# NIH-NEI/oct-image-segmentation-models

Measured on AMD Instinct MI355X. Metric: B-scans/sec (train step), 256x512 3-class U-Net, higher is better.
Workload: dtype f32; 1 GPU; configs[1]: train step (fwd+Dice-macro+bwd+allreduce+Adam), per-GPU batch 32, 256x512x1, 3-class, pool_layers=4, start_neurons=8, random-init weights; global_batch=32, parallelism=dp1, allreduce=none

## Files before the change

oct-image-segmentation-models_amd/csrc/common.hpp:

```cpp
#pragma once
#include <hip/hip_runtime.h>
#include <stdint.h>

namespace oct {

constexpr int kTileX = 32;
constexpr int kTileY = 8;
constexpr int kBlock = 256;

enum { BN_A = 0, BN_B = 1, BN_MEAN = 2, BN_RSTD = 3, BN_C1 = 4, BN_C2 = 5, BN_GA = 6, BN_GB = 7, BN_GD = 8, BN_ARRAYS = 9 };

enum { F_U8 = 1, F_AFF = 2, F_TWO = 4, F_UP = 8, F_DROP = 16 };

static __constant__ float c_u8_lut[256];

__host__ __device__ inline uint32_t drop_hash(uint64_t seed, uint64_t step, uint32_t idx) {
    uint64_t x = seed ^ (step * 0x9E3779B97F4A7C15ull) ^ ((uint64_t)idx * 0xD1B54A32D192ED03ull);
    x ^= x >> 33; x *= 0xff51afd7ed558ccdull;
    x ^= x >> 33; x *= 0xc4ceb9fe1a85ec53ull;
    x ^= x >> 33;
    return (uint32_t)(x >> 32);
}

struct DropCfg {
// ... 101 lines not shown
template <> struct Raw4<float> { using type = float4; };
template <> struct Raw4<bf16_t> { using type = uint2; };
template <typename AT> __device__ inline typename Raw4<AT>::type ldraw4(const AT* p);
template <> __device__ inline float4 ldraw4<float>(const float* p) { return *reinterpret_cast<const float4*>(p); }
template <> __device__ inline uint2 ldraw4<bf16_t>(const bf16_t* p) { return *reinterpret_cast<const uint2*>(p); }
template <typename AT> __device__ inline typename Raw4<AT>::type raw_zero4();
template <> __device__ inline float4 raw_zero4<float>() { return make_float4(0.f, 0.f, 0.f, 0.f); }
template <> __device__ inline uint2 raw_zero4<bf16_t>() { return make_uint2(0u, 0u); }
__device__ inline float4 widen4(const float4& r) { return r; }
__device__ inline float4 widen4(const uint2& u) {
    return make_float4(__uint_as_float(u.x << 16), __uint_as_float(u.x & 0xFFFF0000u),
                       __uint_as_float(u.y << 16), __uint_as_float(u.y & 0xFFFF0000u));
}
template <typename AT> __device__ inline void sta4(AT* p, const float4& v);
template <> __device__ inline void sta4<float>(float* p, const float4& v) { *reinterpret_cast<float4*>(p) = v; }
typedef __bf16 bf16x2_hw __attribute__((ext_vector_type(2)));
typedef float f32x2_hw __attribute__((ext_vector_type(2)));
template <> __device__ inline void sta4<bf16_t>(bf16_t* p, const float4& v) {
    uint2 u;
    u.x = __builtin_bit_cast(uint32_t, __builtin_convertvector(f32x2_hw{v.x, v.y}, bf16x2_hw));
    u.y = __builtin_bit_cast(uint32_t, __builtin_convertvector(f32x2_hw{v.z, v.w}, bf16x2_hw));
    *reinterpret_cast<uint2*>(p) = u;
}
template <typename AT> __device__ inline float lda1(const AT* p);
template <> __device__ inline float lda1<float>(const float* p) { return *p; }
template <> __device__ inline float lda1<bf16_t>(const bf16_t* p) { return bf2f(*p); }

}
```

oct-image-segmentation-models_amd/csrc/host.hpp:

```cpp
#pragma once
#include <hip/hip_runtime.h>

#include <string>
#include <vector>

#include "common.hpp"
#include "kernels_bwd.hpp"
#include "kernels_igemm.hpp"

namespace octh {

struct Options {
    int thin_min_tiles = 2048;
    int dw32_blocks = 512, dw16_blocks = 768;
    int igemm_p_blocks = 1280;
    int igemm_min_blocks = 512;
    int dwpair8 = 1;
    int pair_geo = 221;
    int pair_min_tiles = 2048;
    int dw_side_stream = 1;
    int bx_two_blocks = 1;
    int bx_waves = 8;
    int fuse_first_apply = 1;
    int fuse_bn_apply = 1;
    int fuse_bn_apply16 = 1;
    int fuse_dw_thin = 1;
    int timing_skip = 0;
    int fuse_bn_finalize = 0;
    int bt_m2 = 1;
    int dwbt_f32_all = 0;
    int bt_blocks_per_cu = 0;
    int dwbx_enable = 1;
    int dwbx_blocks = 256;
    int bx_min_blocks = 256;
    int mfma_mode = 1;
    int focal_clip_mod = 0;
    int fork_on_launch = 1;
    int dw_fork_group = 1;
    int event_sysfence = 0;
    int persist_min_tiles = 2048;
};
extern Options g_opt;

int fail(int code, const std::string& msg);

#define HIP_OK(expr)                                                                                      \
    do {                                                                                                  \
        hipError_t e__ = (expr);                                                                          \
        if (e__ != hipSuccess) return ::octh::fail(-5, std::string(#expr) + ": " + hipGetErrorString(e__)); \
    } while (0)

// ... 44 lines not shown
```

oct-image-segmentation-models_amd/csrc/kernels_bwd.hpp:

```cpp
#pragma once
#include "common.hpp"
#include "kernels_fwd.hpp"

namespace oct {

struct PoolBwdArgs {
    const void* gp;
    const void* z;
    const float* bn;
    void* g;
    float* part;
    int H, W, C, tiles_x, tiles, act_bf16;
    FinDesc fin;
};

template <int C_T, typename AT>
__global__ __launch_bounds__(kBlock) void pool_bwd_k(const PoolBwdArgs A) {
    __shared__ float red[256];
    const int Ho = A.H >> 1, Wo = A.W >> 1;
    const int tx = threadIdx.x & (kTileX - 1), ty = threadIdx.x / kTileX;
    const int tile = blockIdx.x;
    const int xo = (tile % A.tiles_x) * kTileX + tx, yo = (tile / A.tiles_x) * kTileY + ty;
    const int b = blockIdx.z, c0 = blockIdx.y * C_T;
    const bool valid = xo < Wo && yo < Ho;
// ... 27 lines not shown
                yv[q] = fmaxf(fmaf(a, zv[q][i], bb), 0.f);
                if (yv[q] > best) { best = yv[q]; am = q; }
            }
#pragma unroll
            for (int q = 0; q < 4; ++q) {
                const float gt = yv[q] > 0.f ? gd[q][i] + (q == am ? gpv[i] : 0.f) : 0.f;
                s1[i] += gt; s2[i] += gt * ((zv[q][i] - mean) * rstd);
                gd[q][i] = gt;
            }
        }
#pragma unroll
        for (int q = 0; q < 4; ++q)
#pragma unroll
            for (int i = 0; i < C_T; i += 4) sta4<AT>(Ag + off[q] + i, make_float4(gd[q][i], gd[q][i + 1], gd[q][i + 2], gd[q][i + 3]));
    }
    float* out = A.part + ((size_t)b * A.tiles + tile) * (2 * A.C);
    block_reduce_store<C_T>(s1, red, out + c0, C_T);
    block_reduce_store<C_T>(s2, red, out + A.C + c0, C_T);
}

template <typename AT, int V = 4>
__global__ __launch_bounds__(kBlock) void pool_bwd_flat_k(const PoolBwdArgs A, int B) {
    static_assert(V == 4 || V == 8, "channels per thread");
    __shared__ float sh[4 * 64 * 8];
    const int CV = A.C / V, Ho = A.H >> 1, Wo = A.W >> 1;
    const size_t n = (size_t)B * Ho * Wo * CV;
    const int tid = threadIdx.x, lane = tid & 63, wave = tid >> 6, c = V * (tid % CV);
    float a[V], bb[V], mean[V], rstd[V], s1[V], s2[V];
#pragma unroll
    for (int k = 0; k < V; ++k) {
        a[k] = A.bn[BN_A * A.C + c + k]; bb[k] = A.bn[BN_B * A.C + c + k];
        mean[k] = A.bn[BN_MEAN * A.C + c + k]; rstd[k] = A.bn[BN_RSTD * A.C + c + k];
        s1[k] = 0.f; s2[k] = 0.f;
    }
    const AT* Az = reinterpret_cast<const AT*>(A.z); AT* Ag = reinterpret_cast<AT*>(A.g);
    const AT* Agp = reinterpret_cast<const AT*>(A.gp);
    for (size_t i = (size_t)blockIdx.x * kBlock + tid; i < n; i += (size_t)gridDim.x * kBlock) {
        size_t r = i / CV;
        const int xo = (int)(r % Wo); r /= Wo;
        const int yo = (int)(r % Ho); const int b = (int)(r / Ho);
        float gpv[V];
        size_t off[4]; float zv[4][V], gd[4][V];
        const size_t goff = (((size_t)b * Ho + yo) * Wo + xo) * A.C + c;
#pragma unroll
        for (int j = 0; j < V; j += 4) {
            const float4 gq = lda4<AT>(Agp + goff + j);
            gpv[j] = gq.x; gpv[j + 1] = gq.y; gpv[j + 2] = gq.z; gpv[j + 3] = gq.w;
// ... 280 lines not shown
#pragma unroll
                for (int kx = 0; kx < KW; ++kx)
                    acc[ky * KW + kx] = fmaf(Xs[((py + ky) * XW + pxx + kx) * CI_T + ci], d, acc[ky * KW + kx]);
        }
    }
#pragma unroll
    for (int k = 0; k < TAPS; ++k) Rs[t * (TAPS + 1) + k] = acc[k];
    Rs[t * (TAPS + 1) + TAPS] = accb;
    __syncthreads();
    if (t < NT) {
        const size_t wsize = (size_t)TAPS * A.Cin * A.Cout;
        float* out = A.part + (size_t)blockIdx.x * (wsize + A.Cout);
        const bool ok = (ci0 + ci < A.Cin) && (co0 + co < A.Cout);
        for (int k = 0; k <= TAPS; ++k) {
            float s = 0.f;
            for (int q = 0; q < PS; ++q) s += Rs[(q * NT + t) * (TAPS + 1) + k];
            if (!ok) continue;
            if (k < TAPS) out[((size_t)k * A.Cin + ci0 + ci) * A.Cout + co0 + co] = s;
            else if (ci0 + ci == 0) out[wsize + co0 + co] = s;
        }
    }
}

template <typename AT, bool FUSE>
__global__ __launch_bounds__(kBlock) void conv_dw_first_k(const ConvBwdWArgs A, int tiles_x, int tiles, int total_tiles) {
    constexpr int TH = 8, TW = 128, XH = TH + 2, XW = TW + 2;
    __shared__ float Xs[XH * XW];
    __shared__ float red[256];
    __shared__ float lut_s[256];
    const int t = threadIdx.x, xl = t & 31, row = t >> 5;
    lut_s[t] = c_u8_lut[t];
    float acc0[64], acc1[16];
#pragma unroll
    for (int k = 0; k < 64; ++k) acc0[k] = 0.f;
#pragma unroll
    for (int k = 0; k < 16; ++k) acc1[k] = 0.f;
    const bool u8 = (A.flags & F_U8) != 0;
    for (int tl = blockIdx.x; tl < total_tiles; tl += gridDim.x) {
        const int b = tl / tiles, tile = tl % tiles;
        const int x0 = (tile % tiles_x) * TW, y0 = (tile / tiles_x) * TH;
        __syncthreads();
        {
            constexpr int NS = (XH * XW + kBlock - 1) / kBlock;
            unsigned int rb[NS]; float rf[NS]; bool in[NS];
#pragma unroll
            for (int k = 0; k < NS; ++k) {
                const int i = t + k * kBlock, cy = i / XW, cx = i % XW, iy = y0 + cy - 1, ix = x0 + cx - 1;
                in[k] = i < XH * XW && iy >= 0 && iy < A.H && ix >= 0 && ix < A.W;
                const size_t pix = in[k] ? ((size_t)b * A.H + iy) * A.W + ix : 0;
                rb[k] = 0; rf[k] = 0.f;
                if (in[k]) { if (u8) rb[k] = reinterpret_cast<const unsigned char*>(A.x0)[pix]; else rf[k] = reinterpret_cast<const float*>(A.x0)[pix]; }
            }
#pragma unroll
            for (int k = 0; k < NS; ++k) {
                const int i = t + k * kBlock;
                if (i < XH * XW) Xs[i] = in[k] ? (u8 ? lut_s[rb[k]] : rf[k]) : 0.f;
            }
        }
        __syncthreads();
        const int y = y0 + row;
#pragma unroll
        for (int k = 0; k < TW / 32; ++k) {
            const int xx = xl + 32 * k, x = x0 + xx;
            if (y < A.H && x < A.W) {
                const size_t e8 = (((size_t)b * A.H + y) * A.W + x) * 8;
                const AT* dp = reinterpret_cast<const AT*>(A.dz) + e8;
                const float4 d0 = lda4<AT>(dp), d1 = lda4<AT>(dp + 4);
                float d[8] = {d0.x, d0.y, d0.z, d0.w, d1.x, d1.y, d1.z, d1.w};
                if constexpr (FUSE) {
                    const AT* zp = reinterpret_cast<const AT*>(A.zf) + e8;
                    const float4 z0 = lda4<AT>(zp), z1 = lda4<AT>(zp + 4);
                    const float zv[8] = {z0.x, z0.y, z0.z, z0.w, z1.x, z1.y, z1.z, z1.w};
#pragma unroll
                    for (int co = 0; co < 8; ++co) {
                        const float o = bn_bwd_apply1(A.bnf[BN_GA * 8 + co], A.bnf[BN_GB * 8 + co], A.bnf[BN_GD * 8 + co], d[co], zv[co]);
                        d[co] = dz_as_stored<AT>(o);
                        asm volatile("" : "+v"(d[co]));
                    }
                }
#pragma unroll
                for (int tap = 0; tap < 9; ++tap) {
                    const float xv = Xs[(row + tap / 3) * XW + xx + tap % 3];
#pragma unroll
                    for (int co = 0; co < 8; ++co) {
                        if (tap < 8) acc0[tap * 8 + co] = fmaf(xv, d[co], acc0[tap * 8 + co]);
                        else acc1[co] = fmaf(xv, d[co], acc1[co]);
                    }
                }
#pragma unroll
                for (int co = 0; co < 8; ++co) acc1[8 + co] += d[co];
            }
        }
    }
    float* out = A.part + (size_t)blockIdx.x * 80;
    block_reduce_store<64>(acc0, red, out, 64);
    block_reduce_store<16>(acc1, red, out + 64, 16);
}

// ... 75 lines not shown
```

oct-image-segmentation-models_amd/csrc/kernels_fin.hpp:

```cpp
#pragma once
#include "common.hpp"

namespace oct {

struct FinDesc {
    unsigned* counter;
    int bwd;
    double count;
    float* bn;
    const float* gamma; const float* beta;
    float* mm; float* mv; float eps, momentum; int unbiased;
    float* dgamma; float* dbeta;
};

__device__ __forceinline__ void bn_fwd_finalize_write(double s, double q, double count, int C, int c, float* __restrict__ bn,
                                                      const float* __restrict__ gamma, const float* __restrict__ beta,
                                                      float* __restrict__ mm, float* __restrict__ mv, float eps, float momentum,
                                                      int unbiased) {
    const double mean = s / count;
    double var = q / count - mean * mean;
    if (var < 0) var = 0;
    const double rstd = 1.0 / sqrt(var + (double)eps);
    const double a = (double)gamma[c] * rstd;
    bn[BN_A * C + c] = (float)a;
    bn[BN_B * C + c] = (float)((double)beta[c] - mean * a);
    bn[BN_MEAN * C + c] = (float)mean;
    bn[BN_RSTD * C + c] = (float)rstd;
    const double m = momentum;
    const double uv = (unbiased && count > 1) ? var * (count / (count - 1.0)) : var;
    mm[c] = (float)((double)mm[c] * m + mean * (1.0 - m));
    mv[c] = (float)((double)mv[c] * m + uv * (1.0 - m));
}

__device__ __forceinline__ void bn_bwd_finalize_write(double s, double q, double count, int C, int c, float* __restrict__ bn,
                                                      const float* __restrict__ gamma, float* __restrict__ dgamma,
                                                      float* __restrict__ dbeta) {
    dbeta[c] = (float)s;
    dgamma[c] = (float)q;
    const double c1 = s / count, c2 = q / count;
    const double rstd = (double)bn[BN_RSTD * C + c], mean = (double)bn[BN_MEAN * C + c];
    const double ga = (double)gamma[c] * rstd, gb = -ga * rstd * c2, gd = -ga * c1 - gb * mean;
    bn[BN_C1 * C + c] = (float)c1; bn[BN_C2 * C + c] = (float)c2;
    bn[BN_GA * C + c] = (float)ga; bn[BN_GB * C + c] = (float)gb; bn[BN_GD * C + c] = (float)gd;
}

__device__ __forceinline__ void part_store(float* p, float v) { __hip_atomic_store(p, v, __ATOMIC_RELAXED, __HIP_MEMORY_SCOPE_AGENT); }

__device__ inline void finalize_in_launch(const FinDesc& F, const float* __restrict__ part, int rows, int C, unsigned nblocks, char* lds) {
    asm volatile("s_waitcnt vmcnt(0)" ::: "memory");
    __syncthreads();
    int* const flag = reinterpret_cast<int*>(lds);
    if (threadIdx.x == 0) {
        const unsigned prev = __hip_atomic_fetch_add(F.counter, 1u, __ATOMIC_RELAXED, __HIP_MEMORY_SCOPE_AGENT);
        *flag = prev == nblocks - 1 ? 1 : 0;
    }
    __syncthreads();
    if (*flag) {
        double* const sh = reinterpret_cast<double*>(lds + 16);
        double* const tot = sh + 2 * (size_t)blockDim.x;
        const int Wp = C, G = (int)blockDim.x / Wp, t = threadIdx.x;
        if (t < G * Wp) {
            const int q = t % Wp, g = t / Wp;
            const unsigned long long* col = reinterpret_cast<const unsigned long long*>(part) + q;
            double s0 = 0, s1 = 0;
            int r = g;
            for (; r + 31 * G < rows; r += 32 * G) {
                unsigned long long v[32];
#pragma unroll
                for (int k = 0; k < 32; ++k) v[k] = __hip_atomic_load(col + (size_t)(r + k * G) * Wp, __ATOMIC_RELAXED, __HIP_MEMORY_SCOPE_AGENT);
#pragma unroll
                for (int k = 0; k < 32; ++k) { s0 += (double)__uint_as_float((unsigned)v[k]); s1 += (double)__uint_as_float((unsigned)(v[k] >> 32)); }
            }
            for (; r + 7 * G < rows; r += 8 * G) {
                unsigned long long v[8];
#pragma unroll
                for (int k = 0; k < 8; ++k) v[k] = __hip_atomic_load(col + (size_t)(r + k * G) * Wp, __ATOMIC_RELAXED, __HIP_MEMORY_SCOPE_AGENT);
// ... 2 lines not shown
            }
            for (; r < rows; r += G) {
                const unsigned long long v = __hip_atomic_load(col + (size_t)r * Wp, __ATOMIC_RELAXED, __HIP_MEMORY_SCOPE_AGENT);
                s0 += (double)__uint_as_float((unsigned)v); s1 += (double)__uint_as_float((unsigned)(v >> 32));
            }
            sh[2 * t] = s0; sh[2 * t + 1] = s1;
        }
        __syncthreads();
        if (t < 2 * C) {
            double a = 0;
            for (int g = 0; g < G; ++g) a += sh[2 * (g * Wp + (t >> 1)) + (t & 1)];
            tot[t] = a;
        }
        __syncthreads();
        if (t < C) {
            if (F.bwd) bn_bwd_finalize_write(tot[t], tot[C + t], F.count, C, t, F.bn, F.gamma, F.dgamma, F.dbeta);
            else bn_fwd_finalize_write(tot[t], tot[C + t], F.count, C, t, F.bn, F.gamma, F.beta, F.mm, F.mv, F.eps, F.momentum, F.unbiased);
        }
        if (t == 0) __hip_atomic_store(F.counter, 0u, __ATOMIC_RELAXED, __HIP_MEMORY_SCOPE_AGENT);
    }
    __syncthreads();
}

}
```

oct-image-segmentation-models_amd/csrc/kernels_fwd.hpp:

```cpp
#pragma once
#include "common.hpp"
#include "kernels_fin.hpp"

namespace oct {

struct ConvFwdArgs {
    const void* x0;
    const float* ab0;
    int C0;
    const float* x1;
    const float* ab1;
    int C1;
    const float* w;
    const float* bias;
    void* z;
    float* part;
    int H, W, Cin, Cout, tiles_x, tiles;
    DropCfg drop;
    int act_bf16;
    FinDesc fin;
};

template <int CO_T, int FLAGS>
__device__ inline void accum_src(const void* __restrict__ src, const float* __restrict__ ab, int C, size_t pix,
// ... 66 lines not shown
            const int sy = UP ? iy >> 1 : iy, sx = UP ? ix >> 1 : ix;
            const size_t pix = inb ? ((size_t)b * Hs + sy) * Ws + sx : 0;
            const float* wk = A.w + (size_t)((ky * KW + kx) * A.Cin) * A.Cout + co0;
            accum_src<CO_T, FLAGS>(A.x0, A.ab0, A.C0, pix, inb, wk, A.Cout, A.drop, acc);
            if constexpr (TWO)
                accum_src<CO_T, FLAGS>(A.x1, A.ab1, A.C1, pix, inb, wk + (size_t)A.C0 * A.Cout, A.Cout, A.drop, acc);
        }
    }
    if (valid) {
        AT* zp = reinterpret_cast<AT*>(A.z) + (((size_t)b * A.H + y) * A.W + x) * A.Cout + co0;
#pragma unroll
        for (int j = 0; j < CO_T; j += 4) sta4<AT>(zp + j, make_float4(acc[j], acc[j + 1], acc[j + 2], acc[j + 3]));
    }
    if (A.part) {
        float s[CO_T], q[CO_T];
#pragma unroll
        for (int j = 0; j < CO_T; ++j) { s[j] = valid ? acc[j] : 0.f; q[j] = s[j] * s[j]; }
        float* out = A.part + ((size_t)b * A.tiles + tile) * (2 * A.Cout);
        block_reduce_store<CO_T>(s, red, out + co0, CO_T);
        block_reduce_store<CO_T>(q, red, out + A.Cout + co0, CO_T);
    }
}

template <typename AT>
__global__ __launch_bounds__(kBlock) void conv_first_fwd_k(const ConvFwdArgs A, int x_is_u8, int tiles_x, int tiles, int total_tiles,
                                                          const float* __restrict__ wgt, const float* __restrict__ bias) {
    constexpr int TH = 8, TW = 128, XH = TH + 2, XW = TW + 2;
    __shared__ float Xs[XH * XW];
    __shared__ float red[256];
    __shared__ float lut_s[256];
    const int t = threadIdx.x, xl = t & 31, row = t >> 5;
    lut_s[t] = c_u8_lut[t];
    float s1[8], s2[8];
#pragma unroll
    for (int j = 0; j < 8; ++j) { s1[j] = 0.f; s2[j] = 0.f; }
    for (int tl = blockIdx.x; tl < total_tiles; tl += gridDim.x) {
        const int b = tl / tiles, tile = tl % tiles;
        const int x0 = (tile % tiles_x) * TW, y0 = (tile / tiles_x) * TH;
        __syncthreads();
        {
            constexpr int NS = (XH * XW + kBlock - 1) / kBlock;
            unsigned int rb[NS]; float rf[NS]; bool in[NS];
#pragma unroll
            for (int k = 0; k < NS; ++k) {
                const int i = t + k * kBlock, cy = i / XW, cx = i % XW, iy = y0 + cy - 1, ix = x0 + cx - 1;
                in[k] = i < XH * XW && iy >= 0 && iy < A.H && ix >= 0 && ix < A.W;
                const size_t pix = in[k] ? ((size_t)b * A.H + iy) * A.W + ix : 0;
                rb[k] = 0; rf[k] = 0.f;
                if (in[k]) { if (x_is_u8) rb[k] = reinterpret_cast<const unsigned char*>(A.x0)[pix]; else rf[k] = reinterpret_cast<const float*>(A.x0)[pix]; }
            }
#pragma unroll
            for (int k = 0; k < NS; ++k) {
                const int i = t + k * kBlock;
                if (i < XH * XW) Xs[i] = in[k] ? (x_is_u8 ? lut_s[rb[k]] : rf[k]) : 0.f;
            }
        }
        __syncthreads();
        const int y = y0 + row;
#pragma unroll
        for (int k = 0; k < TW / 32; ++k) {
            const int xx = xl + 32 * k, x = x0 + xx;
            float acc[8];
#pragma unroll
            for (int j = 0; j < 8; ++j) acc[j] = bias[j];
#pragma unroll
            for (int tap = 0; tap < 9; ++tap) {
                const float xv = Xs[(row + tap / 3) * XW + xx + tap % 3];
#pragma unroll
                for (int j = 0; j < 8; ++j) acc[j] = fmaf(xv, wgt[tap * 8 + j], acc[j]);
            }
            if (y < A.H && x < A.W) {
                AT* zp = reinterpret_cast<AT*>(A.z) + (((size_t)b * A.H + y) * A.W + x) * 8;
                sta4<AT>(zp, make_float4(acc[0], acc[1], acc[2], acc[3]));
                sta4<AT>(zp + 4, make_float4(acc[4], acc[5], acc[6], acc[7]));
#pragma unroll
                for (int j = 0; j < 8; ++j) { s1[j] += acc[j]; s2[j] = fmaf(acc[j], acc[j], s2[j]); }
            }
        }
    }
    if (A.part) {
        float* out = A.part + (size_t)blockIdx.x * 16;
        block_reduce_store<8, true>(s1, red, out, 8);
        block_reduce_store<8, true>(s2, red, out + 8, 8);
        if (A.fin.counter) finalize_in_launch(A.fin, A.part, gridDim.x, 8, gridDim.x, reinterpret_cast<char*>(Xs));
    }
}

struct BnFinArgs {
    const float* part;
    int nblk, C;
    double count;
    const float* gamma; const float* beta;
    float* bn;
// ... 84 lines not shown
}

template <int C, int CIN>
__device__ inline void head_logits(const float* __restrict__ ab, const float* __restrict__ w, const float* __restrict__ bias,
                                   float (&y)[CIN], const float (&zr)[CIN], float (&p)[C]) {
#pragma unroll
    for (int i = 0; i < CIN; ++i) y[i] = fmaxf(fmaf(ab[i], zr[i], ab[CIN + i]), 0.f);
    float mx = -3.4e38f;
#pragma unroll
    for (int c = 0; c < C; ++c) {
        float l = bias[c];
#pragma unroll
        for (int i = 0; i < CIN; ++i) l = fmaf(y[i], w[i * C + c], l);
        p[c] = l; mx = fmaxf(mx, l);
    }
    float sum = 0.f;
#pragma unroll
    for (int c = 0; c < C; ++c) { p[c] = expf(p[c] - mx); sum += p[c]; }
    const float inv = 1.f / sum;
#pragma unroll
    for (int c = 0; c < C; ++c) p[c] *= inv;
}

template <int C, int CIN, typename AT>
__global__ __launch_bounds__(kBlock) void head_fwd_k(const HeadFwdArgs A) {
    constexpr int N = DiceN<C>::value;
    __shared__ float red[256];
    const int b = blockIdx.y;
    float v[N];
#pragma unroll
    for (int i = 0; i < N; ++i) v[i] = 0.f;
    for (int chunk = blockIdx.x; chunk * kBlock < A.HW; chunk += gridDim.x) {
        const int px = chunk * kBlock + threadIdx.x;
        const bool valid = px < A.HW;
        const size_t pix = (size_t)b * A.HW + (valid ? px : 0);
        float y[CIN], zr[CIN], p[C];
        head_load<CIN, AT>(reinterpret_cast<const AT*>(A.z) + pix * CIN, zr);
        head_logits<C, CIN>(A.ab, A.w, A.bias, y, zr, p);
        if (valid) {
            if (A.probs) {
#pragma unroll
                for (int c = 0; c < C; ++c) A.probs[pix * C + c] = p[c];
            }
            if (A.argmax) {
                int am = 0; float best = p[0];
#pragma unroll
                for (int c = 1; c < C; ++c) if (p[c] > best) { best = p[c]; am = c; }
                A.argmax[pix] = (unsigned char)am;
            }
            if (A.labels) {
                const int lab = A.labels[pix];
#pragma unroll
                for (int c = 0; c < C; ++c) {
                    const float yv = lab == c ? 1.f : 0.f, ph = p[c] > 0.5f ? 1.f : 0.f;
                    v[c * kDiceVals + 0] += yv * p[c]; v[c * kDiceVals + 1] += yv; v[c * kDiceVals + 2] += p[c];
                    v[c * kDiceVals + 3] += yv * ph;   v[c * kDiceVals + 4] += ph;
                }
                if (A.focal_on) {
                    float py = p[0];
#pragma unroll
                    for (int c = 1; c < C; ++c) py = lab == c ? p[c] : py;
// ... 113 lines not shown
```

oct-image-segmentation-models_amd/csrc/oct_unet.hip:

```cpp
#include <hip/hip_runtime.h>
#include <hip/hip_ext.h>

#include <cmath>
#include <cstdio>
#include <cstring>
#include <string>
#include <vector>

#include "../../include/oct_unet.h"
#include "host.hpp"
#include "kernels_bwd.hpp"
#include "kernels_fwd.hpp"
#include "kernels_igemm.hpp"
#include "kernels_bx.hpp"

using namespace oct;
using namespace octh;

#ifndef OCT_SRC_HASH
#define OCT_SRC_HASH "unstamped"
#endif

namespace octh {
Options g_opt;
// ... 247 lines not shown
    return off;
}

DropCfg make_drop(const oct_unet* h) {
    DropCfg d;
    d.seed = h->cfg.seed; d.step = h->drop_step;
    const double r = h->cfg.dropout_rate;
    d.thresh = (unsigned)std::min(4294967295.0, std::floor(r * 4294967296.0));
    d.scale = (float)(1.0 / (1.0 - r));
    return d;
}

inline bool fin_ok(const oct_unet* h, const Layer& l) { return h->opt.fuse_bn_finalize && l.has_bn && l.cout <= 32 && l.cout % 2 == 0; }
FinDesc fin_desc(const oct_unet* h, int li, int bwd, int B) {
    const Layer& l = h->plan.L[li];
    FinDesc f{};
    f.counter = h->fin_counters + 2 * li + (bwd ? 1 : 0); f.bwd = bwd; f.count = (double)B * l.H * l.W;
    f.bn = l.bn; f.gamma = h->params + l.gamma_off; f.beta = h->params + l.beta_off;
    f.mm = h->state + l.mm_off; f.mv = h->state + l.mv_off;
    f.eps = h->cfg.bn_eps; f.momentum = h->cfg.bn_momentum; f.unbiased = h->cfg.bn_unbiased_moving_var;
    if (bwd) { f.dgamma = h->grads + l.gamma_off; f.dbeta = h->grads + l.beta_off; }
    return f;
}

template <int KH, int FLAGS>
int launch_conv_fwd_co(const ConvFwdArgs& a, int B, hipStream_t s, const char* layer, double flops, double bytes) {
    const int co_t = chunk_of(a.Cout);
    dim3 grid(a.tiles, a.Cout / co_t, B), block(kBlock);
    char nm[64]; snprintf(nm, sizeof nm, "conv_fwd_k<%d,%d,%d,%s>", KH, co_t, FLAGS, AT_NAME(a.act_bf16));
    ProfScope ps(s, nm, layer, flops, bytes);
    switch (co_t) {
        case 16: AT_DISPATCH(a.act_bf16, conv_fwd_k<KH, 16, FLAGS, AT><<<grid, block, 0, s>>>(a)); break;
        case 8: AT_DISPATCH(a.act_bf16, conv_fwd_k<KH, 8, FLAGS, AT><<<grid, block, 0, s>>>(a)); break;
        default: AT_DISPATCH(a.act_bf16, conv_fwd_k<KH, 4, FLAGS, AT><<<grid, block, 0, s>>>(a)); break;
    }
    HIP_OK(hipGetLastError());
    return 0;
}

struct SrcDesc { const void* x0; const float* ab0; int C0; const void* x1; const float* ab1; int C1; int flags; };

SrcDesc src_of(const oct_unet* h, int li, const void* x_in, int x_is_u8) {
    const Layer& l = h->plan.L[li];
    SrcDesc d{}; d.x1 = nullptr; d.ab1 = nullptr; d.C1 = 0;
    switch (l.src) {
        case SRC_INPUT: d.x0 = x_in; d.ab0 = nullptr; d.C0 = l.cin; d.flags = x_is_u8 ? F_U8 : 0; break;
// ... 210 lines not shown
    e.jw = e.stride < 16384 ? 16 : 64;
    e.blk_start = R.n ? R.L[R.n - 1].blk_start + cdiv((int)R.L[R.n - 1].stride, R.L[R.n - 1].jw) : 0;
    ++R.n;
}

int flush_reduce(oct_unet* h, hipStream_t s) {
    ReduceAllArgs& R = h->red;
    if (!R.n) return 0;
    const ReduceAllArgs::Entry& last = R.L[R.n - 1];
    const unsigned blocks = last.blk_start + cdiv((int)last.stride, last.jw);
    double bytes = 0;
    for (int i = 0; i < R.n; ++i) bytes += (double)R.L[i].npb * R.L[i].stride * 4;
    ProfScope ps(s, "reduce_all_k", "all", 0, bytes);
    reduce_all_k<<<blocks, kBlock, 0, s>>>(R);
    HIP_OK(hipGetLastError());
    R.n = 0;
    return 0;
}

inline bool first_dw_streams(const Layer& l) {
    return l.src == SRC_INPUT && l.cin == 1 && l.cout == 8 && l.kh == 3 && l.has_bn && !l.drop_in;
}

int conv_backward_w(oct_unet* h, int li, const void* x_in, int x_is_u8, const void* dz, int B, hipStream_t s, bool fused_apply) {
    const Layer& l = h->plan.L[li];
    const Options& o = h->opt;
    const SrcDesc sd = src_of(h, li, x_in, x_is_u8);
    DwPlan p = dw_plan(l, B, o.mfma_mode, h->cfg.dtype, o);
    p.npb = std::min(p.npb, l.dw_rows);
    ConvBwdWArgs a{};
    a.x0 = sd.x0; a.ab0 = sd.ab0; a.C0 = sd.C0; a.x1 = sd.x1; a.ab1 = sd.ab1; a.C1 = sd.C1;
    a.flags = sd.flags | (l.drop_in ? F_DROP : 0);
    a.dz = dz; a.part = l.dwp;
    a.B = B; a.H = l.H; a.W = l.W; a.Cin = l.cin; a.Cout = l.cout;
    a.tiles_x = cdiv(l.W, kTileX); a.tiles = p.tiles; a.total_tiles = B * a.tiles; a.npb = p.npb;
    a.drop = make_drop(h); a.act_bf16 = h->cfg.dtype;
    if (fused_apply) { a.zf = l.z; a.bnf = l.bn; }
    const double px = (double)B * l.H * l.W, fl = 2.0 * l.kh * l.kw * l.cin * l.cout * px;
    const int es = h->cfg.dtype ? 2 : 4;
    const double by = in_bytes(l, B, x_is_u8, es) + px * l.cout * es * (fused_apply ? 2 : 1);
    const bool up = l.src == SRC_UP;
    const LaunchCtx lc{&o, B, s, l.name, fl, by};
    int rc = 0;
    if (p.kind == 0 && l.cin == 1 && l.cout == 8 && l.kh == 3 && !(a.flags & (F_AFF | F_DROP | F_TWO | F_UP))) {
        const int tx = cdiv(l.W, 128), tiles = tx * cdiv(l.H, 8), total = B * tiles;
        const int grid = std::min(total, a.npb);
        a.npb = grid;
        const int bf = a.act_bf16;
        ProfScope ps(s, bf ? "conv_dw_first_k<unsigned short>" : "conv_dw_first_k<float>", l.name, fl, by);
        if (fused_apply) AT_DISPATCH(bf, (conv_dw_first_k<AT, true><<<grid, kBlock, 0, s>>>(a, tx, tiles, total)));
        else AT_DISPATCH(bf, (conv_dw_first_k<AT, false><<<grid, kBlock, 0, s>>>(a, tx, tiles, total)));
        HIP_OK(hipGetLastError());
    } else if (p.kind == 0) {
        if (fused_apply) return fail(-3, "conv_backward_w: the generic first-layer kernel does not apply the BN-backward transform");
        rc = launch_dw<3>(a, p.cic, p.coc, s, l.name, fl, by);
    } else if (p.kind == 33 || p.kind == 34) {
        rc = launch_dw_bf16pipe(a, p, l.kh, up, lc);
    } else {
        rc = launch_dw_f32pipe(a, p, l.kh, up, lc);
    }
    if (rc) return rc;
    queue_reduce(h, l, a.npb);
    return 0;
}

int bn_backward(oct_unet* h, int li, int nblk, int B, hipStream_t s, bool finalize_only, bool finalized_in_launch,
                hipEvent_t done = nullptr, bool* bound = nullptr) {
    const Layer& l = h->plan.L[li];
    if (bound) *bound = false;
    if (!finalized_in_launch && !(h->opt.timing_skip & 2 && h->drop_step > 2)) {
        BnBwdFinArgs f{};
        f.part = h->stat_part; f.nblk = nblk; f.C = l.cout; f.count = (double)B * l.H * l.W;
        f.bn = l.bn; f.gamma = h->params + l.gamma_off; f.dgamma = h->grads + l.gamma_off; f.dbeta = h->grads + l.beta_off;
        ProfScope ps(s, "bn_bwd_finalize_k", l.name, 0, (double)nblk * 2 * l.cout * 4);
        if (done && finalize_only) {
            hipExtLaunchKernelGGL(bn_bwd_finalize_k, dim3(l.cout), dim3(kBlock), 0, s, nullptr, done, 0, f);
// ... 95 lines not shown
            fuse = o.fuse_first_apply && li == 0 && first_dw_streams(l) && dwkind == 0 &&
                   !(src_of(h, li, x_in, x_is_u8).flags & (F_AFF | F_DROP | F_TWO | F_UP));
        } else {
            const int cg = bx_bwd_cg(l);
            const bool up = l.src == SRC_UP;
            const ConvRoute r0 = conv_route(dx_args(nullptr, cg, 0, nullptr, up), up ? A_DOWN2 : A_NORMAL, o);
            fuse = o.fuse_bn_apply && dwkind != 0 && r0 != ROUTE_F32 && !(up && r0 == ROUTE_BX && l.cout > kBxGbDown2MaxC) &&
                   !(r0 == ROUTE_BT && l.cout == 32) && !(r0 == ROUTE_BT && l.cout == 16 && cg == 16 && !o.fuse_bn_apply16) &&
                   (l.src != SRC_CONCAT || conv_route(dx_args(nullptr, cg, cg, nullptr, false), A_NORMAL, o) != ROUTE_F32);
        }
        l.g_masked = fuse;
        bool fdw = false;
        if (fuse && o.fuse_dw_thin && l.kh == 3 && l.cout == 8 && !l.drop_in && (l.src == SRC_PREV || l.src == SRC_CONCAT) &&
            bx_bwd_cg(l) == 8 && l.dw_rows >= std::min(B * cdiv(l.W, 32) * cdiv(l.H, 8), 512) &&
            conv_route(dx_args(nullptr, 8, 0, nullptr, false), A_NORMAL, o) == ROUTE_BT &&
            (l.src != SRC_CONCAT || conv_route(dx_args(nullptr, 8, 8, nullptr, false), A_NORMAL, o) == ROUTE_BT))
            fdw = true;
        const bool fork = side_ok && !fdw && l.src != SRC_INPUT;
        const bool tail_here = li == first_mid_layer(pl);
        if (fork) pend.push_back({li, fuse});
        const bool flush = !pend.empty() && (!fork || (int)pend.size() >= o.dw_fork_group || tail_here);
        hipEvent_t fe = flush ? h->fork_ev[1 + n_forks++ % (h->fork_ev.size() - 1)] : nullptr;
        bool fe_bound = false;
        rc = bn_backward(h, li, pending_nblk, B, s, fuse, pending_fin, (flush && o.fork_on_launch) ? fe : nullptr, &fe_bound);
        if (rc) return rc;
        pending_fin = false;
        if (flush) {
            if (!fe_bound) HIP_OK(hipEventRecord(fe, s));
            HIP_OK(hipStreamWaitEvent(h->side, fe, 0));
            for (const PendingDw& p : pend) {
                rc = conv_backward_w(h, p.li, x_in, x_is_u8, pl.L[p.li].g, B, h->side, p.fuse);
                if (rc) return rc;
            }
            pend.clear();
            forked = true;
        }
        if (!fdw && !fork) {
            rc = conv_backward_w(h, li, x_in, x_is_u8, l.g, B, s, fuse);
            if (rc) return rc;
        }
        if (tail_here && (forked || h->tail_event)) {
            hipStream_t rs = forked ? h->side : s;
            rc = flush_reduce(h, rs);
            if (rc) return rc;
            if (h->tail_event) HIP_OK(hipEventRecord(h->tail_event, rs));
        }
        if (l.src == SRC_INPUT) break;
        if (prep_pending) { HIP_OK(hipStreamWaitEvent(s, h->prep_ev, 0)); prep_pending = false; }
        int rows = 0;
        auto dx = [&](void* gout, int Cg, int ci_off, const Layer* prod, bool up, const Layer* xsrc = nullptr, bool first = true) -> int {
            IgemmArgs g = dx_args(gout, Cg, ci_off, prod, up);
            if (fuse) { g.gb_z = l.z; g.gb_bn = l.bn; }
            const double px = (double)B * l.H * l.W, pxg = (double)B * g.Ho * g.Wo;
            double fl = 2.0 * l.kh * l.kw * Cg * l.cout * px;
            const int es = h->cfg.dtype ? 2 : 4;
            double by = px * l.cout * es * (fuse ? 2 : 1) + pxg * Cg * es * (prod ? 2 : 1);
            if (fdw) {
                g.dw_x = xsrc->z; g.dw_ab = xsrc->bn; g.dw_part = l.dwp; g.dw_Cin = l.cin; g.dw_ci_off = ci_off; g.dw_bias = first ? 1 : 0;
                fl *= 2; if (!prod) by += pxg * Cg * es;
            }
            const LaunchCtx lc{&o, B, s, l.name, fl, by};
// ... 400 lines not shown
    const size_t n = (size_t)B * H * W;
    boundary_maps_k<<<(int)std::min<size_t>((n + kBlock - 1) / kBlock, 8192), kBlock, 0, (hipStream_t)stream>>>(
        labels, maps, B, H, W, n_cls, bg_ilm, bg_csi);
    HIP_OK(hipGetLastError());
    return 0;
}

namespace {
struct Opt { const char* name; int Options::*var; int lo, hi; };
const Opt k_opts[] = {
    {"igemm_persistent_min_tiles", &Options::persist_min_tiles, 1, 1 << 30}, {"dw32_blocks", &Options::dw32_blocks, 64, 1 << 20},
    {"dw16_blocks", &Options::dw16_blocks, 64, 1 << 20}, {"igemm_persistent_blocks", &Options::igemm_p_blocks, 8, 1 << 20},
    {"igemm_min_blocks", &Options::igemm_min_blocks, 1, 1 << 30}, {"dwpair8_enable", &Options::dwpair8, 0, 1},
    {"pair8_geometry", &Options::pair_geo, 111, 221}, {"pair8_min_tiles", &Options::pair_min_tiles, 1, 1 << 30},
    {"thin8_min_tiles", &Options::thin_min_tiles, 1, 1 << 30}, {"focal_clip_modulation", &Options::focal_clip_mod, 0, 1},
    {"mfma_mode", &Options::mfma_mode, 0, 1}, {"bx_min_blocks", &Options::bx_min_blocks, 1, 1 << 30},
    {"dwbx_blocks", &Options::dwbx_blocks, 8, 1 << 20}, {"bt_blocks_per_cu", &Options::bt_blocks_per_cu, 0, 8},
    {"dwbt_f32_all", &Options::dwbt_f32_all, 0, 1}, {"bt_m2", &Options::bt_m2, 0, 1},
    {"fuse_first_apply", &Options::fuse_first_apply, 0, 1}, {"fuse_bn_apply", &Options::fuse_bn_apply, 0, 1},
    {"fuse_bn_finalize", &Options::fuse_bn_finalize, 0, 1}, {"bx_waves", &Options::bx_waves, 4, 8},
    {"dw_side_stream", &Options::dw_side_stream, 0, 1}, {"timing_skip", &Options::timing_skip, 0, 255}, {"fuse_dw_thin", &Options::fuse_dw_thin, 0, 1},
    {"dwbx_enable", &Options::dwbx_enable, 0, 1},
    {"bx_two_blocks", &Options::bx_two_blocks, 0, 1}, {"fork_on_launch", &Options::fork_on_launch, 0, 1},
    {"event_sysfence", &Options::event_sysfence, 0, 1}, {"dw_fork_group", &Options::dw_fork_group, 1, 8}, {"fuse_bn_apply16", &Options::fuse_bn_apply16, 0, 1},
};
}

int oct_get_option(const char* name, int* value) {
    if (!name || !value) return fail(-1, "null argument");
    for (const Opt& o : k_opts) if (!strcmp(name, o.name)) { *value = g_opt.*o.var; return 0; }
    return fail(-1, std::string("unknown option: ") + name);
}

int oct_set_option(const char* name, int value) {
    if (!name) return fail(-1, "null option name");
    if (!strcmp(name, "pair8_geometry") && value != 221 && value != 111) return fail(-1, "pair8_geometry must be 221 or 111");
    if (!strcmp(name, "bx_waves") && value != 4 && value != 8) return fail(-1, "bx_waves must be 4 or 8");
    for (const Opt& o : k_opts)
        if (!strcmp(name, o.name)) { g_opt.*o.var = value < o.lo ? o.lo : (value > o.hi ? o.hi : value); return 0; }
    return fail(-1, std::string("unknown option: ") + name);
}

int oct_unet_get_option(const oct_unet* h, const char* name, int* value) {
    if (!h || !name || !value) return fail(-1, "null argument");
    for (const Opt& o : k_opts) if (!strcmp(name, o.name)) { *value = h->opt.*o.var; return 0; }
    return fail(-1, std::string("unknown option: ") + name);
// ... 25 lines not shown
```

Baseline: 8367 B-scans/s.

## Recompute first-layer conv output in weight-grad kernel instead of reloading z

In the first-layer weight-gradient kernel with fused BN-backward, the pre-BN activation z is now recomputed from the input tile already held in shared memory (9 taps x 8 channels) instead of being read from global memory. This is on by default and removes one full-resolution 8-channel activation read. It also adds an off-by-default option that finalizes BN statistics inside the consumer kernel, and hoists the head weights into registers. The cost is extra FMAs per pixel, plus rounding to bf16 to match the stored values.

```diff
diff --git a/oct-image-segmentation-models_amd/csrc/common.hpp b/oct-image-segmentation-models_amd/csrc/common.hpp
--- a/oct-image-segmentation-models_amd/csrc/common.hpp
+++ b/oct-image-segmentation-models_amd/csrc/common.hpp
@@ -147,6 +147,14 @@
     u.y = __builtin_bit_cast(uint32_t, __builtin_convertvector(f32x2_hw{v.z, v.w}, bf16x2_hw));
     *reinterpret_cast<uint2*>(p) = u;
 }
+template <typename AT> __device__ inline float4 as_stored4(const float4& v);
+template <> __device__ inline float4 as_stored4<float>(const float4& v) { return v; }
+template <> __device__ inline float4 as_stored4<bf16_t>(const float4& v) {
+    const uint32_t x = __builtin_bit_cast(uint32_t, __builtin_convertvector(f32x2_hw{v.x, v.y}, bf16x2_hw));
+    const uint32_t y = __builtin_bit_cast(uint32_t, __builtin_convertvector(f32x2_hw{v.z, v.w}, bf16x2_hw));
+    return make_float4(__uint_as_float(x << 16), __uint_as_float(x & 0xFFFF0000u),
+                       __uint_as_float(y << 16), __uint_as_float(y & 0xFFFF0000u));
+}
 template <typename AT> __device__ inline float lda1(const AT* p);
 template <> __device__ inline float lda1<float>(const float* p) { return *p; }
 template <> __device__ inline float lda1<bf16_t>(const bf16_t* p) { return bf2f(*p); }
diff --git a/oct-image-segmentation-models_amd/csrc/host.hpp b/oct-image-segmentation-models_amd/csrc/host.hpp
--- a/oct-image-segmentation-models_amd/csrc/host.hpp
+++ b/oct-image-segmentation-models_amd/csrc/host.hpp
@@ -27,6 +27,8 @@
     int fuse_dw_thin = 1;
     int timing_skip = 0;
     int fuse_bn_finalize = 0;
+    int first_dw_recompute_z = 1;
+    int fin_in_consumer = 0;
     int bt_m2 = 1;
     int dwbt_f32_all = 0;
     int bt_blocks_per_cu = 0;
diff --git a/oct-image-segmentation-models_amd/csrc/kernels_bwd.hpp b/oct-image-segmentation-models_amd/csrc/kernels_bwd.hpp
--- a/oct-image-segmentation-models_amd/csrc/kernels_bwd.hpp
+++ b/oct-image-segmentation-models_amd/csrc/kernels_bwd.hpp
@@ -73,7 +73,7 @@
 template <typename AT, int V = 4>
 __global__ __launch_bounds__(kBlock) void pool_bwd_flat_k(const PoolBwdArgs A, int B) {
     static_assert(V == 4 || V == 8, "channels per thread");
-    __shared__ float sh[4 * 64 * 8];
+    __shared__ __attribute__((aligned(16))) float sh[4 * 64 * 8];
     const int CV = A.C / V, Ho = A.H >> 1, Wo = A.W >> 1;
     const size_t n = (size_t)B * Ho * Wo * CV;
     const int tid = threadIdx.x, lane = tid & 63, wave = tid >> 6, c = V * (tid % CV);
@@ -400,14 +400,27 @@
     }
 }
 
-template <typename AT, bool FUSE>
-__global__ __launch_bounds__(kBlock) void conv_dw_first_k(const ConvBwdWArgs A, int tiles_x, int tiles, int total_tiles) {
+template <typename AT, bool FUSE, bool RECOMP = false, bool FINC = false>
+__global__ __launch_bounds__(kBlock) void conv_dw_first_k(const ConvBwdWArgs A, int tiles_x, int tiles, int total_tiles,
+                                                         const float* __restrict__ wgt, const float* __restrict__ bias,
+                                                         const FinDesc fin, const float* __restrict__ fin_part, int fin_rows) {
+    static_assert(FUSE || !(RECOMP || FINC), "z and the record are only needed where the transform is applied");
     constexpr int TH = 8, TW = 128, XH = TH + 2, XW = TW + 2;
     __shared__ float Xs[XH * XW];
     __shared__ float red[256];
     __shared__ float lut_s[256];
+    __shared__ __attribute__((aligned(16))) char fin_lds[FINC ? kFinConsumerLds : 16];
     const int t = threadIdx.x, xl = t & 31, row = t >> 5;
     lut_s[t] = c_u8_lut[t];
+    float bnf[24];
+    if constexpr (FINC) {
+        const float* cf = finalize_in_consumer(fin, fin_part, fin_rows, 8, fin_lds, blockIdx.x == 0);
+#pragma unroll
+        for (int k = 0; k < 24; ++k) bnf[k] = cf[k];
+    } else if constexpr (FUSE) {
+#pragma unroll
+        for (int k = 0; k < 24; ++k) bnf[k] = A.bnf[BN_GA * 8 + k];
+    }
     float acc0[64], acc1[16];
 #pragma unroll
     for (int k = 0; k < 64; ++k) acc0[k] = 0.f;
@@ -446,12 +459,20 @@
                 const float4 d0 = lda4<AT>(dp), d1 = lda4<AT>(dp + 4);
                 float d[8] = {d0.x, d0.y, d0.z, d0.w, d1.x, d1.y, d1.z, d1.w};
                 if constexpr (FUSE) {
-                    const AT* zp = reinterpret_cast<const AT*>(A.zf) + e8;
-                    const float4 z0 = lda4<AT>(zp), z1 = lda4<AT>(zp + 4);
+                    float4 z0, z1;
+                    if constexpr (RECOMP) {
+                        float zr[8];
+                        first_conv_px<XW>(Xs + row * XW + xx, wgt, bias, zr);
+                        z0 = as_stored4<AT>(make_float4(zr[0], zr[1], zr[2], zr[3]));
+                        z1 = as_stored4<AT>(make_float4(zr[4], zr[5], zr[6], zr[7]));
+                    } else {
+                        const AT* zp = reinterpret_cast<const AT*>(A.zf) + e8;
+                        z0 = lda4<AT>(zp); z1 = lda4<AT>(zp + 4);
+                    }
                     const float zv[8] = {z0.x, z0.y, z0.z, z0.w, z1.x, z1.y, z1.z, z1.w};
 #pragma unroll
                     for (int co = 0; co < 8; ++co) {
-                        const float o = bn_bwd_apply1(A.bnf[BN_GA * 8 + co], A.bnf[BN_GB * 8 + co], A.bnf[BN_GD * 8 + co], d[co], zv[co]);
+                        const float o = bn_bwd_apply1(bnf[co], bnf[8 + co], bnf[16 + co], d[co], zv[co]);
                         d[co] = dz_as_stored<AT>(o);
                         asm volatile("" : "+v"(d[co]));
                     }
diff --git a/oct-image-segmentation-models_amd/csrc/kernels_fin.hpp b/oct-image-segmentation-models_amd/csrc/kernels_fin.hpp
--- a/oct-image-segmentation-models_amd/csrc/kernels_fin.hpp
+++ b/oct-image-segmentation-models_amd/csrc/kernels_fin.hpp
@@ -32,16 +32,27 @@
     mv[c] = (float)((double)mv[c] * m + uv * (1.0 - m));
 }
 
+struct BnBwdCoef { float dbeta, dgamma, c1, c2, ga, gb, gd; };
+__device__ __forceinline__ BnBwdCoef bn_bwd_coef(double s, double q, double count, float gamma, float rstd_f, float mean_f) {
+    BnBwdCoef r;
+    r.dbeta = (float)s; r.dgamma = (float)q;
+    const double c1 = s / count, c2 = q / count;
+    const double rstd = (double)rstd_f, mean = (double)mean_f;
+    const double ga = (double)gamma * rstd, gb = -ga * rstd * c2, gd = -ga * c1 - gb * mean;
+    r.c1 = (float)c1; r.c2 = (float)c2; r.ga = (float)ga; r.gb = (float)gb; r.gd = (float)gd;
+    return r;
+}
+__device__ __forceinline__ void bn_bwd_record_write(const BnBwdCoef& k, int C, int c, float* __restrict__ bn,
+                                                    float* __restrict__ dgamma, float* __restrict__ dbeta) {
+    dbeta[c] = k.dbeta;
+    dgamma[c] = k.dgamma;
+    bn[BN_C1 * C + c] = k.c1; bn[BN_C2 * C + c] = k.c2;
+    bn[BN_GA * C + c] = k.ga; bn[BN_GB * C + c] = k.gb; bn[BN_GD * C + c] = k.gd;
+}
 __device__ __forceinline__ void bn_bwd_finalize_write(double s, double q, double count, int C, int c, float* __restrict__ bn,
                                                       const float* __restrict__ gamma, float* __restrict__ dgamma,
                                                       float* __restrict__ dbeta) {
-    dbeta[c] = (float)s;
-    dgamma[c] = (float)q;
-    const double c1 = s / count, c2 = q / count;
-    const double rstd = (double)bn[BN_RSTD * C + c], mean = (double)bn[BN_MEAN * C + c];
-    const double ga = (double)gamma[c] * rstd, gb = -ga * rstd * c2, gd = -ga * c1 - gb * mean;
-    bn[BN_C1 * C + c] = (float)c1; bn[BN_C2 * C + c] = (float)c2;
-    bn[BN_GA * C + c] = (float)ga; bn[BN_GB * C + c] = (float)gb; bn[BN_GD * C + c] = (float)gd;
+    bn_bwd_record_write(bn_bwd_coef(s, q, count, gamma[c], bn[BN_RSTD * C + c], bn[BN_MEAN * C + c]), C, c, bn, dgamma, dbeta);
 }
 
 __device__ __forceinline__ void part_store(float* p, float v) { __hip_atomic_store(p, v, __ATOMIC_RELAXED, __HIP_MEMORY_SCOPE_AGENT); }
@@ -51,7 +62,7 @@
     __syncthreads();
     int* const flag = reinterpret_cast<int*>(lds);
     if (threadIdx.x == 0) {
-        const unsigned prev = __hip_atomic_fetch_add(F.counter, 1u, __ATOMIC_RELAXED, __HIP_MEMORY_SCOPE_AGENT);
+        const unsigned prev = __hip_atomic_fetch_add(F.counter, 1u, __ATOMIC_ACQ_REL, __HIP_MEMORY_SCOPE_AGENT);
         *flag = prev == nblocks - 1 ? 1 : 0;
     }
     __syncthreads();
@@ -100,4 +111,47 @@
     __syncthreads();
 }
 
+constexpr int kFinConsumerLds = 4 * 64 * 8 + 64 * 8 + 96 * 4;
+__device__ inline const float* finalize_in_consumer(const FinDesc& F, const float* __restrict__ part, int rows, int C, char* lds,
+                                                    bool write_record) {
+    double* const wsum = reinterpret_cast<double*>(lds);
+    double* const tot = wsum + 4 * 64;
+    float* const coef = reinterpret_cast<float*>(tot + 64);
+    const int t = threadIdx.x, Q = C >> 1, G = kBlock / Q;
+    const int cq = t % Q, g = t / Q;
+    double s[4] = {0, 0, 0, 0};
+    const unsigned ld = 2 * (unsigned)C;
+    unsigned e = (unsigned)g * ld + 4 * cq;
+    const unsigned end = (unsigned)rows * ld, step = (unsigned)G * ld;
+    for (; e < end; e += 8 * step) {
+        float4 v[8];
+#pragma unroll
+        for (int k = 0; k < 8; ++k) {
+            const unsigned ek = e + k * step;
+            v[k] = ek < end ? *reinterpret_cast<const float4*>(part + ek) : make_float4(0.f, 0.f, 0.f, 0.f);
+        }
+#pragma unroll
+        for (int k = 0; k < 8; ++k) { s[0] += (double)v[k].x; s[1] += (double)v[k].y; s[2] += (double)v[k].z; s[3] += (double)v[k].w; }
+    }
+    for (int o = 32; o >= Q; o >>= 1) {
+#pragma unroll
+        for (int j = 0; j < 4; ++j) s[j] += __shfl_xor(s[j], o, 64);
+    }
+    const int lane = t & 63, wave = t >> 6;
+    if (lane < Q) {
+#pragma unroll
+        for (int j = 0; j < 4; ++j) wsum[wave * 64 + 4 * lane + j] = s[j];
+    }
+    __syncthreads();
+    if (t < 2 * C) tot[t] = (wsum[t] + wsum[64 + t]) + (wsum[128 + t] + wsum[192 + t]);
+    __syncthreads();
+    if (t < C) {
+        const BnBwdCoef k = bn_bwd_coef(tot[t], tot[C + t], F.count, F.gamma[t], F.bn[BN_RSTD * C + t], F.bn[BN_MEAN * C + t]);
+        coef[t] = k.ga; coef[C + t] = k.gb; coef[2 * C + t] = k.gd;
+        if (write_record) bn_bwd_record_write(k, C, t, F.bn, F.dgamma, F.dbeta);
+    }
+    __syncthreads();
+    return coef;
 }
+
+}
diff --git a/oct-image-segmentation-models_amd/csrc/kernels_fwd.hpp b/oct-image-segmentation-models_amd/csrc/kernels_fwd.hpp
--- a/oct-image-segmentation-models_amd/csrc/kernels_fwd.hpp
+++ b/oct-image-segmentation-models_amd/csrc/kernels_fwd.hpp
@@ -112,6 +112,19 @@
     }
 }
 
+template <int XW>
+__device__ __forceinline__ void first_conv_px(const float* xw, const float* __restrict__ wgt, const float* __restrict__ bias,
+                                              float (&acc)[8]) {
+#pragma unroll
+    for (int j = 0; j < 8; ++j) acc[j] = bias[j];
+#pragma unroll
+    for (int tap = 0; tap < 9; ++tap) {
+        const float xv = xw[(tap / 3) * XW + tap % 3];
+#pragma unroll
+        for (int j = 0; j < 8; ++j) acc[j] = fmaf(xv, wgt[tap * 8 + j], acc[j]);
+    }
+}
+
 template <typename AT>
 __global__ __launch_bounds__(kBlock) void conv_first_fwd_k(const ConvFwdArgs A, int x_is_u8, int tiles_x, int tiles, int total_tiles,
                                                           const float* __restrict__ wgt, const float* __restrict__ bias) {
@@ -151,14 +164,7 @@
         for (int k = 0; k < TW / 32; ++k) {
             const int xx = xl + 32 * k, x = x0 + xx;
             float acc[8];
-#pragma unroll
-            for (int j = 0; j < 8; ++j) acc[j] = bias[j];
-#pragma unroll
-            for (int tap = 0; tap < 9; ++tap) {
-                const float xv = Xs[(row + tap / 3) * XW + xx + tap % 3];
-#pragma unroll
-                for (int j = 0; j < 8; ++j) acc[j] = fmaf(xv, wgt[tap * 8 + j], acc[j]);
-            }
+            first_conv_px<XW>(Xs + row * XW + xx, wgt, bias, acc);
             if (y < A.H && x < A.W) {
                 AT* zp = reinterpret_cast<AT*>(A.z) + (((size_t)b * A.H + y) * A.W + x) * 8;
                 sta4<AT>(zp, make_float4(acc[0], acc[1], acc[2], acc[3]));
@@ -289,11 +295,25 @@
     for (int c = 0; c < C; ++c) p[c] *= inv;
 }
 
+template <int N>
+__device__ __forceinline__ void load_uniform(const float* __restrict__ p, float (&r)[N]) {
+#pragma unroll
+    for (int i = 0; i < N; ++i) r[i] = p[i];
+}
+__host__ __device__ constexpr bool head_hoist_ok(int C, int CIN) { return 4 * CIN + CIN * C + C <= 64; }
+
 template <int C, int CIN, typename AT>
 __global__ __launch_bounds__(kBlock) void head_fwd_k(const HeadFwdArgs A) {
     constexpr int N = DiceN<C>::value;
     __shared__ float red[256];
     const int b = blockIdx.y;
+    constexpr bool HOIST = head_hoist_ok(C, CIN);
+    float abr[HOIST ? 2 * CIN : 1], wr[HOIST ? CIN * C : 1], br[HOIST ? C : 1];
+    const float* ab = A.ab; const float* w = A.w; const float* bias = A.bias;
+    if constexpr (HOIST) {
+        load_uniform(A.ab, abr); load_uniform(A.w, wr); load_uniform(A.bias, br);
+        ab = abr; w = wr; bias = br;
+    }
     float v[N];
 #pragma unroll
     for (int i = 0; i < N; ++i) v[i] = 0.f;
@@ -303,7 +323,7 @@
         const size_t pix = (size_t)b * A.HW + (valid ? px : 0);
         float y[CIN], zr[CIN], p[C];
         head_load<CIN, AT>(reinterpret_cast<const AT*>(A.z) + pix * CIN, zr);
-        head_logits<C, CIN>(A.ab, A.w, A.bias, y, zr, p);
+        head_logits<C, CIN>(ab, w, bias, y, zr, p);
         if (valid) {
             if (A.probs) {
 #pragma unroll
diff --git a/oct-image-segmentation-models_amd/csrc/oct_unet.hip b/oct-image-segmentation-models_amd/csrc/oct_unet.hip
--- a/oct-image-segmentation-models_amd/csrc/oct_unet.hip
+++ b/oct-image-segmentation-models_amd/csrc/oct_unet.hip
@@ -293,6 +293,8 @@
     if (bwd) { f.dgamma = h->grads + l.gamma_off; f.dbeta = h->grads + l.beta_off; }
     return f;
 }
+
+constexpr size_t kFinConsumerMaxBytes = 64 * 1024;
 
 template <int KH, int FLAGS>
 int launch_conv_fwd_co(const ConvFwdArgs& a, int B, hipStream_t s, const char* layer, double flops, double bytes) {
@@ -549,7 +551,8 @@
     return l.src == SRC_INPUT && l.cin == 1 && l.cout == 8 && l.kh == 3 && l.has_bn && !l.drop_in;
 }
 
-int conv_backward_w(oct_unet* h, int li, const void* x_in, int x_is_u8, const void* dz, int B, hipStream_t s, bool fused_apply) {
+int conv_backward_w(oct_unet* h, int li, const void* x_in, int x_is_u8, const void* dz, int B, hipStream_t s, bool fused_apply,
+                    bool finc = false, int finc_rows = 0) {
     const Layer& l = h->plan.L[li];
     const Options& o = h->opt;
     const SrcDesc sd = src_of(h, li, x_in, x_is_u8);
@@ -565,7 +568,8 @@
     if (fused_apply) { a.zf = l.z; a.bnf = l.bn; }
     const double px = (double)B * l.H * l.W, fl = 2.0 * l.kh * l.kw * l.cin * l.cout * px;
     const int es = h->cfg.dtype ? 2 : 4;
-    const double by = in_bytes(l, B, x_is_u8, es) + px * l.cout * es * (fused_apply ? 2 : 1);
+    const bool recomp = fused_apply && o.first_dw_recompute_z && first_dw_streams(l);
+    const double by = in_bytes(l, B, x_is_u8, es) + px * l.cout * es * (fused_apply && !recomp ? 2 : 1);
     const bool up = l.src == SRC_UP;
     const LaunchCtx lc{&o, B, s, l.name, fl, by};
     int rc = 0;
@@ -575,10 +579,18 @@
         a.npb = grid;
         const int bf = a.act_bf16;
         ProfScope ps(s, bf ? "conv_dw_first_k<unsigned short>" : "conv_dw_first_k<float>", l.name, fl, by);
-        if (fused_apply) AT_DISPATCH(bf, (conv_dw_first_k<AT, true><<<grid, kBlock, 0, s>>>(a, tx, tiles, total)));
-        else AT_DISPATCH(bf, (conv_dw_first_k<AT, false><<<grid, kBlock, 0, s>>>(a, tx, tiles, total)));
+        const float* w = h->params + l.w_off; const float* bias = h->params + l.b_off;
+        FinDesc fin{};
+        if (finc) { fin = fin_desc(h, li, 1, B); fin.counter = nullptr; }
+        const float* fpart = h->stat_part;
+#define DW_FIRST(FUSE, RECOMP, FINC) AT_DISPATCH(bf, (conv_dw_first_k<AT, FUSE, RECOMP, FINC><<<grid, kBlock, 0, s>>>(a, tx, tiles, total, w, bias, fin, fpart, finc_rows)))
+        if (!fused_apply) { if (finc) return fail(-3, "conv_backward_w: statistics can only be finalized where the transform is applied"); DW_FIRST(false, false, false); }
+        else if (recomp) { if (finc) DW_FIRST(true, true, true); else DW_FIRST(true, true, false); }
+        else { if (finc) DW_FIRST(true, false, true); else DW_FIRST(true, false, false); }
+#undef DW_FIRST
         HIP_OK(hipGetLastError());
     } else if (p.kind == 0) {
+        if (finc) return fail(-3, "conv_backward_w: only the streaming first-layer kernel finalizes statistics");
         if (fused_apply) return fail(-3, "conv_backward_w: the generic first-layer kernel does not apply the BN-backward transform");
         rc = launch_dw<3>(a, p.cic, p.coc, s, l.name, fl, by);
     } else if (p.kind == 33 || p.kind == 34) {
@@ -720,7 +732,9 @@
         const bool flush = !pend.empty() && (!fork || (int)pend.size() >= o.dw_fork_group || tail_here);
         hipEvent_t fe = flush ? h->fork_ev[1 + n_forks++ % (h->fork_ev.size() - 1)] : nullptr;
         bool fe_bound = false;
-        rc = bn_backward(h, li, pending_nblk, B, s, fuse, pending_fin, (flush && o.fork_on_launch) ? fe : nullptr, &fe_bound);
+        const bool finc0 = o.fin_in_consumer && !o.timing_skip && l.src == SRC_INPUT && fuse && !pending_fin && !fork &&
+                           (size_t)pending_nblk * 2 * l.cout * 4 <= kFinConsumerMaxBytes;
+        rc = bn_backward(h, li, pending_nblk, B, s, fuse, pending_fin || finc0, (flush && o.fork_on_launch) ? fe : nullptr, &fe_bound);
         if (rc) return rc;
         pending_fin = false;
         if (flush) {
@@ -734,7 +748,7 @@
             forked = true;
         }
         if (!fdw && !fork) {
-            rc = conv_backward_w(h, li, x_in, x_is_u8, l.g, B, s, fuse);
+            rc = conv_backward_w(h, li, x_in, x_is_u8, l.g, B, s, fuse, finc0, pending_nblk);
             if (rc) return rc;
         }
         if (tail_here && (forked || h->tail_event)) {
@@ -1181,6 +1195,7 @@
     {"dw_side_stream", &Options::dw_side_stream, 0, 1}, {"timing_skip", &Options::timing_skip, 0, 255}, {"fuse_dw_thin", &Options::fuse_dw_thin, 0, 1},
     {"dwbx_enable", &Options::dwbx_enable, 0, 1},
     {"bx_two_blocks", &Options::bx_two_blocks, 0, 1}, {"fork_on_launch", &Options::fork_on_launch, 0, 1},
+    {"first_dw_recompute_z", &Options::first_dw_recompute_z, 0, 1}, {"fin_in_consumer", &Options::fin_in_consumer, 0, 1},
     {"event_sysfence", &Options::event_sysfence, 0, 1}, {"dw_fork_group", &Options::dw_fork_group, 1, 8}, {"fuse_bn_apply16", &Options::fuse_bn_apply16, 0, 1},
 };
 }
```

After: 8447 B-scans/s, median of 6. About the same (+1.0%).
